# AlenkaF/vaex

Measured on AMD Instinct MI355X. Metric: rows/sec 2D count grid 1e9×f64 + groupby-sum 1e6 keys; HBM GB/s %peak, higher is better.
Workload: dtype f64; 1 GPU; C2 (BASELINE configs[1]): count(binby=[x,y], limits=[[-4,4],[-4,4]], shape=1024) + sum(w), one merged pass; rows_per_gpu=1000000000, parallelism=row-shard x1

## Files before the change

vaex_amd/csrc/engine.hpp:

```cpp
#pragma once
#include <memory>
#include <mutex>
#include <vector>

#include "common.hpp"
#include "hashset.hpp"

struct vh_grid;
struct vh_agg;


namespace vh {

constexpr int MAX_DIM = 16;
constexpr int MAX_FUSED_AGGS = 4;
constexpr uint64_t LDS_FUSED_MAX = 64 * 1024;
constexpr uint64_t LDS_AGG_MAX_BYTES = 96 * 1024;
constexpr int COV_MAX_N = 8;

struct ColumnRef {
    const void *ptr = nullptr;
    uint64_t size = 0;
    int itemsize = 0;
    int loc = VH_LOC_HOST;
// ... 122 lines not shown
    std::vector<int> isz;
    std::vector<uint64_t> off;
    uint64_t chunk = 0, bytes = 0;
    PinnedBuf pinned[2];
    DevBuf dev[2];
    hipEvent_t copied[2] = {nullptr, nullptr}, consumed[2] = {nullptr, nullptr};
    bool pending_copy[2] = {false, false}, pending_use[2] = {false, false};
    std::vector<void *> registered[2];
    ~HostPipe();
    void release_registered(int b);
    void add(const ColumnRef &c);
    void plan(uint64_t chunk_rows);
    void issue(uint64_t ci, uint64_t row0, uint64_t len);
    void wait_copied(int b);
    void mark_consumed(int b);
    int find(const void *ptr) const;
};

struct Workspace {
    DevBuf idx;
    DevBuf cells;
    DevBuf first_part;
    HostPipe pipe;
    ~Workspace();
};

void run_bin(vh_grid *g, vh_agg *const *aggs, int naggs, uint64_t length);
void launch_fused(const BinPlan &plan, FusedAggs &fa, uint64_t n, uint64_t cells, int nd_f64, Workspace &ws);
bool try_tiled(const BinPlan &plan, const FusedAggs &fa, uint64_t n, uint64_t cells, int nd_f64, Workspace &ws);
uint64_t stat_tile_overflow(bool reset);
uint64_t stat_hashagg_overflow(bool reset);
uint64_t stat_set_overflow(bool reset);
uint64_t stat_tile_stream_rounds(bool reset);
bool try_tiled_first(const BinPlan &plan, const AggDev &ad, uint64_t n, uint64_t cells, uint64_t row0, int nd_f64);
uint64_t stat_first_tiled(bool reset);
bool hashagg_bin_set_ordinal(const BinPlan &plan, const FusedAggs &fa, uint64_t n);

}

struct vh_grid {
    std::mutex mu;
    std::vector<vh_binner *> binners;
    std::vector<uint64_t> shapes, strides;
    uint64_t length1d = 1;
    vh::Workspace ws;
};

struct vh_agg {
    vh_grid *grid = nullptr;
    int kind = 0, dtype = VH_F64, flip = 0;
    uint32_t moment = 0;
    int grid_dtype = VH_I64;
    int grid_isz = 8;
    vh::DevBuf g, g2;
    vh::DevBuf s_key, s_row;
    vh::ColumnRef data, data2, mask;
    vh::ColumnRef cols[vh::COV_MAX_N];
    bool has_selection = false;
    bool nu_dirty = false;
    uint64_t L = 0;
    uint64_t nu_n = 0;
    vh::DevBuf nu_cell, nu_val;
};

namespace vh {
void nunique_init(vh_agg *a);
// ... 18 lines not shown
```

vaex_amd/csrc/runtime.hip:

```cpp
#include <map>
#include <mutex>
#include <thread>
#include <cstring>

#include "common.hpp"
#include "engine.hpp"

namespace vh {

static thread_local std::string g_last_error;

void set_error_str(const std::string &s) { g_last_error = s; }
void set_error(const char *fmt, ...) {
    char buf[1024];
    va_list ap;
    va_start(ap, fmt);
    vsnprintf(buf, sizeof(buf), fmt, ap);
    va_end(ap);
    g_last_error = buf;
}

static std::mutex g_mu;
static std::map<int, hipStream_t> g_streams;
static std::map<int, int> g_cus;
// ... 699 lines not shown
    VH_HIP(hipStreamSynchronize(stream()));
    std::lock_guard<std::mutex> lk(g_mu);
    for (auto &kv : g_timing_recs)
        for (auto &p : kv.second.ev) {
            (void)hipEventDestroy(p.first);
            (void)hipEventDestroy(p.second);
        }
    g_timing_recs.clear();
    VH_API_END
}

int vh_timing_read(const char *kernel, uint64_t *launches, double *total_ms) {
    VH_API_BEGIN
    VH_HIP(hipStreamSynchronize(stream()));
    std::lock_guard<std::mutex> lk(g_mu);
    *launches = 0;
    *total_ms = 0;
    auto it = g_timing_recs.find(kernel);
    if (it == g_timing_recs.end()) return VH_OK;
    for (auto &p : it->second.ev) {
        float ms = 0;
        VH_HIP(hipEventElapsedTime(&ms, p.first, p.second));
        *total_ms += ms;
        *launches += 1;
    }
    VH_API_END
}

int vh_stat_read(const char *name, uint64_t *value, int reset) {
    VH_API_BEGIN
    const std::string n = name ? name : "";
    if (n == "tile_overflow_rows") *value = stat_tile_overflow(reset != 0);
    else if (n == "tile_stream_rounds") *value = stat_tile_stream_rounds(reset != 0);
    else if (n == "hashagg_overflow_rows") *value = stat_hashagg_overflow(reset != 0);
    else if (n == "set_overflow_rows") *value = stat_set_overflow(reset != 0);
    else if (n == "first_tiled_chunks") *value = stat_first_tiled(reset != 0);
    else fail(VH_ERR_ARG, "vh_stat_read: unknown statistic '" + n + "'");
    VH_API_END
}

int vh_stream(void **s) {
    VH_API_BEGIN
    *s = (void *)stream();
    VH_API_END
}

static void minmax_result(const DevBuf &keys, double *out_min, double *out_max) {
    thread_local PinnedBuf res_buf;
    res_buf.ensure(16);
    uint64_t *res = res_buf.as<uint64_t>();
    VH_HIP(hipMemcpyAsync(res, keys.ptr, 16, hipMemcpyDeviceToHost, stream()));
    VH_HIP(hipStreamSynchronize(stream()));
    if (res[0] == ~0ULL) {
        *out_min = __builtin_nan("");
        *out_max = __builtin_nan("");
    } else {
        *out_min = f64_from_key(res[0]);
        *out_max = f64_from_key(res[1]);
    }
}

int vh_minmax_sample(const void *data, uint64_t n, int dtype, uint64_t nsample, double *out_min, double *out_max) {
    VH_API_BEGIN
    if (resolve_loc(data, VH_LOC_AUTO) != VH_LOC_DEVICE) throw std::runtime_error("vh_minmax_sample: column not in device memory");
    if (dtype == VH_BOOL) throw std::runtime_error("vh_minmax_sample: bool column");
    const uint64_t ns = std::min(n, nsample);
// ... 67 lines not shown
```

vaex_amd/csrc/tile_plan.hpp:

```cpp
#pragma once
#include <algorithm>
#include <cmath>
#include <vector>

#include "engine.hpp"

namespace vh {

#ifndef VH_TA_THREADS
#define VH_TA_THREADS 512
#endif
#ifndef VH_TA_RPT
#define VH_TA_RPT 8
#endif
#ifndef VH_TB_THREADS
#define VH_TB_THREADS 1024
#endif
#ifndef VH_TILE_LDS_KB
#define VH_TILE_LDS_KB 96
#endif
constexpr int TA_THREADS = VH_TA_THREADS;
constexpr int TA_RPT = VH_TA_RPT;
constexpr int TA_BATCH = TA_THREADS * TA_RPT;
constexpr int TB_THREADS = VH_TB_THREADS;
// ... 42 lines not shown
}

inline bool aligned16(const void *p) { return (reinterpret_cast<uintptr_t>(p) & 15) == 0; }
inline bool aligned8(const void *p) { return (reinterpret_cast<uintptr_t>(p) & 7) == 0; }

struct TileParams {
    uint32_t s_log2, ntiles, flags_mode, nvals;
    uint64_t cells;
    uint32_t W;
    uint32_t pad;
    uint64_t rows_per_wg;
    uint64_t wg_stride;
    const uint32_t *cap;
    const uint64_t *toff;
    uint32_t *fills;
    uint32_t *spill_fill;
    const uint32_t *spill_cap;
    const uint64_t *spill_start;
    uint64_t spill_base;
    void *entries;
    double *values[2];
    int32_t val_slot[MAX_FUSED_AGGS];
    int32_t cnt_slot[MAX_FUSED_AGGS];
    const double *vdata[2];
    uint32_t debug;
    uint32_t vnarrow, vfloat, vsigned;
    uint32_t vpacked;
    int32_t vdt[2];
    void *mmtmp[MAX_FUSED_AGGS];
    uint32_t mgeneric, mmk;
    uint32_t wide, lds_cap;
    uint32_t mm_simple, mm_cnt_nn;
    int32_t mm_off[4];
    uint32_t stream, ncw;
    uint32_t *tab;
    const uint8_t *rowmask;
};

struct TileSwitches {
    bool rowmask = true, f32 = true, narrow = true, stream = true, pack = true;
    uint32_t wide = 7;
    uint64_t wgpad = 0;
    uint32_t debug = 0;
};

struct PassAKernel {
    enum Family { GENERIC, FAST, ORDINAL };
    Family family = GENERIC;
    int nd = 0, nv = 0, sb = 1, ct = VH_F64, vt = VH_F64, dt0 = VH_F64, dt1 = VH_F64;
    bool mk = false, set = false, vn = false;
    const char *scope() const {
        if (family == GENERIC) return "tile_scatter";
        if (family == ORDINAL) return set ? "tile_scatter_set" : "tile_scatter_ord";
        if (ct == VH_I32 || ct == VH_I64) return "tile_scatter_int";
        return ct != vt ? "tile_scatter_mixed" : ct == VH_F32 ? "tile_scatter_f32" : "tile_scatter_f64";
    }
};
const void *pass_a_kernel(const PassAKernel &k);

struct PassBKernel { int nv = 0; bool narrow = false, mm = false, pk = false, mg = false; };
const void *pass_b_kernel(const PassBKernel &k);

struct TilePlan {
    TileParams tp;
    uint32_t lds_off[MAX_FUSED_AGGS];
    uint64_t lds_a, lds_b;
    int sb, vbytes;
    PassAKernel a;
    PassBKernel b;
};

inline bool ord_fast_ok(const BinPlan &plan, const FusedAggs &fa) {
    if (plan.nb != 1) return false;
    const BinnerDev &b = plan.b[0];
    const bool set_ok = b.kind == 2 && (b.dtype == VH_I32 || b.dtype == VH_U32) && !b.set.wide;
    if (!(b.kind == 1 && b.dtype == VH_I32) && !set_ok) return false;
    if (b.flip || b.mask || (reinterpret_cast<uintptr_t>(b.data) & 7)) return false;
    for (int k = 0; k < fa.na; k++) {
        const FusedAgg &a = fa.a[k];
        if (a.mask) return false;
        if (a.kind != VH_AGG_COUNT) {
            if (!a.data) return false;
            const int isz = a.dtype == VH_F64 ? 16 : 2 * dtype_itemsize(a.dtype);
            if (reinterpret_cast<uintptr_t>(a.data) % isz) return false;
        } else if (a.data) {
            bool keyed = false;
            for (int j = 0; j < fa.na; j++)
                if (fa.a[j].kind != VH_AGG_COUNT && fa.a[j].data == a.data) keyed = true;
            if (!keyed) return false;
        }
    }
    return true;
}

// ... 167 lines not shown
    tp.lds_cap = wide ? cap0 + 8 * T : cap0;
    out.lds_a = any_fast ? fast_lds_bytes(nv, T, tp.lds_cap, out.vbytes) : scatter_lds_bytes(nv, T);
    if (out.lds_a > LDS_MAX_BYTES) return false;
    tp.vpacked = (out.vbytes == 4 && nv == 2 && !flags_mode && sw.pack) ? 1u : 0u;

    bool mm = false;
    for (int k = 0; k < fa.na; k++) {
        const FusedAgg &a = fa.a[k];
        mm = mm || is_minmax(a.kind) || a.kind == VH_AGG_SUM_MOMENT;
        if (a.kind == VH_AGG_SUM_MOMENT && a.moment != 2) tp.mgeneric = 1;
        if (is_minmax(a.kind)) tp.mmk |= 1u << k;
    }
    bool simple = mm && !tp.mgeneric && nv == 1 && !vnarrow && !flags_mode;
    int *moff = tp.mm_off;
    moff[0] = moff[1] = moff[2] = moff[3] = -1;
    for (int k = 0; k < fa.na && simple; k++) {
        const FusedAgg &a = fa.a[k];
        const int slot = a.kind == VH_AGG_COUNT ? -1 : tp.val_slot[k];
        int r = -1;
        if (a.kind == VH_AGG_COUNT) {
            r = 0;
            if (tp.cnt_slot[k] == 0) tp.mm_cnt_nn = 1;
            else if (tp.cnt_slot[k] != CNT_ALWAYS) simple = false;
        } else if (a.kind == VH_AGG_SUM && !a.vint && a.dtype == VH_F64 && slot == 0) r = 1;
        else if (a.kind == VH_AGG_MIN && a.dtype == VH_F64 && slot == 0) r = 2;
        else if (a.kind == VH_AGG_MAX && a.dtype == VH_F64 && slot == 0) r = 3;
        else simple = false;
        if (r >= 0) {
            if (moff[r] >= 0) simple = false;
            else moff[r] = (int)out.lds_off[k];
        }
    }
    tp.mm_simple = simple ? 1u : 0u;
    out.b.nv = nv, out.b.pk = nv == 2 && tp.vpacked, out.b.narrow = nv > 0 && (vnarrow || out.b.pk);
    out.b.mm = nv > 0 && mm, out.b.mg = out.b.mm && tp.mgeneric;
    check_pass_a(plan, fa, out);
    return true;
}

struct MetaLayout {
    uint64_t hist;
    uint64_t toff, sstart, scap, sfill, cap;
    uint64_t fills, units, brange;
    uint64_t bytes;
};
struct TileLaunch {
    uint32_t W = 0;
    uint64_t kbat = 0, rows_per_wg = 0, ncw = 0;
    bool stream_layout = false;
    uint64_t stream_stride = 0;
    uint64_t g_min = 1, max_units = 0;
    uint64_t sblocks = 0, bstride = 0;
    MetaLayout meta;
};

inline TileLaunch plan_launch(const TilePlan &pl, uint64_t n, int cus, int blocks_per_cu, const TileSwitches &sw) {
    TileLaunch L;
    const uint32_t T = pl.tp.ntiles;
    const int bpc = std::max(1, std::min(blocks_per_cu, TA_WG_PER_CU));
    const uint32_t W = L.W = std::min<uint32_t>(1024, (uint32_t)cus * bpc);
    const uint64_t nb = (n + TA_BATCH - 1) / TA_BATCH;
    L.kbat = (nb + W - 1) / W;
    L.rows_per_wg = L.kbat * TA_BATCH;
    L.ncw = (L.kbat + pl.sb - 1) / pl.sb;
    L.stream_layout = pl.tp.wide && pl.tp.nvals > 0 && sw.stream && (uint64_t)W * (T + 1) * L.ncw < (1ull << 31);
    L.stream_stride = ((L.rows_per_wg + 7 * L.ncw * T + 8 + 7) & ~uint64_t(7)) + ((sw.wgpad + 7) & ~uint64_t(7));
    const uint64_t wpu = std::max<uint64_t>(1, (uint64_t)TB_THREADS * TB_ROUNDS / std::max<uint64_t>(L.ncw, 1));
    L.g_min = L.stream_layout ? (W + wpu - 1) / wpu : 1;
    L.max_units = (uint64_t)T * L.g_min + 4 * (uint64_t)cus + 16;
    L.sblocks = std::min<uint64_t>(nb, SAMPLE_BLOCKS);
    L.bstride = std::max<uint64_t>(TA_BATCH, n / L.sblocks);
    MetaLayout &m = L.meta;
    uint64_t o = 0;
    auto take = [&](uint64_t bytes) { const uint64_t at = o; o += bytes; return at; };
    m.hist = take(16 * (uint64_t)T);
    m.toff = take(8 * (uint64_t)T);
    m.sstart = take(8 * (uint64_t)T);
    m.scap = take(4 * (uint64_t)T);
    m.sfill = take(4 * (uint64_t)T);
    m.cap = take(4 * (uint64_t)((T + 3) & ~3u));
    m.fills = take(4 * ((uint64_t)T * W + 4 - ((uint64_t)T * W) % 4));
    m.units = take(sizeof(WorkUnit) * L.max_units);
    m.brange = take(8 * (uint64_t)SAMPLE_BLOCKS);
    m.bytes = o;
    return L;
}

inline bool sample_monotone(const uint32_t *brange, uint64_t sblocks) {
    uint64_t up = 0, down = 0;
    for (uint64_t b = 0; b + 1 < sblocks; b++) {
        up += brange[2 * b + 1] > brange[2 * b + 2];
        down += brange[2 * b] < brange[2 * b + 3];
    }
    return sblocks > 8 && std::min(up, down) * 100 <= sblocks;
}

struct TileRegions {
    std::vector<uint32_t> cap, scap;
    std::vector<uint64_t> toff, sstart;
    uint64_t stride = 0, stotal = 0, sampled = 0;
};

inline bool size_regions(const TilePlan &pl, const TileLaunch &L, uint64_t n, const uint64_t *hist, const uint32_t *brange,
                         TileRegions &r) {
    const uint32_t T = pl.tp.ntiles, W = L.W;
    const uint64_t rows_per_wg = L.rows_per_wg, kbat = L.kbat;
    const bool wide = pl.tp.wide != 0, monotone = sample_monotone(brange, L.sblocks);
    uint64_t sampled = 0;
    for (uint32_t t = 0; t < T; t++) sampled += hist[t];
    r.sampled = sampled;
    if (!sampled) return false;
    const uint64_t pad_wg = wide ? 7 * L.ncw : 0;
    r.cap.assign(T, 0), r.scap.assign(T, 0);
    r.toff.assign(T, 0), r.sstart.assign(T, 0);
    uint64_t stride = 0, stotal = 0;
    const double blocks = (double)L.sblocks;
    bool any_clustered = false;
    for (uint32_t t = 0; t < T; t++) {
        const double m = (double)hist[t] / blocks, var_b = std::max(0.0, (double)hist[T + t] / blocks - m * m);
        any_clustered = any_clustered || var_b > 4.0 * m + 1.0;
// ... 78 lines not shown
```

vaex_amd/csrc/tiled.hip:

```cpp
#include <algorithm>
#include <atomic>
#include <cstdio>
#include <cstring>
#include <cmath>
#include <map>
#include <memory>
#include <mutex>
#include <tuple>

#include "binner_dev.hpp"
#include "common.hpp"
#include "engine.hpp"
#include "tile_plan.hpp"

namespace vh {

#ifndef VH_TA_WAVES
#define VH_TA_WAVES 0
#endif
#ifndef VH_TA_NT
#define VH_TA_NT 0
#endif
#ifndef VH_TA_DRAIN
#define VH_TA_DRAIN 1
// ... 1222 lines not shown
    }
}

template <int NV, bool X = false> struct TileRun {
    uint32_t cnt, nn[NV > 0 ? NV : 1];
    double sum[NV > 0 ? NV : 1];
    unsigned long long isum[NV > 0 ? NV : 1];
    double sum2[X && NV > 0 ? NV : 1];
    __device__ void clear() {
        cnt = 0;
#pragma unroll
        for (int s = 0; s < NV; s++) {
            nn[s] = 0;
            sum[s] = 0.0;
            isum[s] = 0;
            if constexpr (X) sum2[s] = 0.0;
        }
    }
    __device__ __attribute__((always_inline)) void add(const TileParams &tp, const double *v) {
        cnt++;
#pragma unroll
        for (int s = 0; s < NV; s++) {
            isum[s] += __builtin_bit_cast(unsigned long long, v[s]);
            if (v[s] == v[s]) {
                nn[s]++;
                sum[s] += v[s];
                if constexpr (X) sum2[s] += v[s] * v[s];
            }

        }
    }
    __device__ __attribute__((always_inline)) void flush(const FusedAggs &fa, const TileParams &tp, unsigned char *lds,
                                                         uint32_t local) const {
#pragma unroll
        for (int k = 0; k < MAX_FUSED_AGGS; k++) {
            if (k >= fa.na) break;
            const int kind = fa.a[k].kind;
            if (kind == VH_AGG_COUNT) {
                const int cs = tp.cnt_slot[k];
                uint32_t c = cs == CNT_ALWAYS || cs == CNT_FLAG ? cnt : 0u;
#pragma unroll
                for (int s = 0; s < NV; s++)
                    if (s == cs) c = nn[s];
                if (c) atomicAdd(reinterpret_cast<uint32_t *>(lds + fa.a[k].lds_off) + local, c);
                continue;
            }
#pragma unroll
            for (int s = 0; s < NV; s++) {
                if (s != tp.val_slot[k]) continue;
                if constexpr (X) {
                    if (kind == VH_AGG_SUM_MOMENT) {
                        if (nn[s]) atomicAdd(reinterpret_cast<double *>(lds + fa.a[k].lds_off) + local, sum2[s]);
                        continue;
                    }
                    if (is_minmax(kind)) continue;
                }
                if (fa.a[k].vint)
                    atomicAdd(reinterpret_cast<unsigned long long *>(lds + fa.a[k].lds_off) + local, isum[s]);
                else if (nn[s])
                    atomicAdd(reinterpret_cast<double *>(lds + fa.a[k].lds_off) + local, sum[s]);
            }
        }
    }
};

constexpr int TB_UNROLL = 8;
// ... 307 lines not shown
#pragma unroll
                                        for (int k = 0; k < MAX_FUSED_AGGS; k++) {
                                            if (!((tp.mmk >> k) & 1u)) continue;
                                            const FusedAgg &a = fa.a[k];
                                            const bool m = a.kind == VH_AGG_MAX;
#pragma unroll
                                            for (int s = 0; s < NV; s++) {
                                                if (s != tp.val_slot[k]) continue;
                                                const uint64_t o = m ? hi[s] : lo[s];
                                                if (o == (m ? 0ull : ~0ull)) continue;
                                                const double r = mm_unokey(a.dtype, o);
                                                if (mm_cell32(a.dtype))
                                                    mm_lds32<false>(reinterpret_cast<uint32_t *>(lds_raw + a.lds_off) + local, a.dtype, m, r);
                                                else
                                                    mm_lds<false>(reinterpret_cast<uint64_t *>(lds_raw + a.lds_off) + local, a.dtype, m, r);
                                            }
                                        }
                                    }
                                }
                            }
                            w0 = (w0 >> 16) | (w1 << 16);
                            w1 = (w1 >> 16) | (w2 << 16);
                            w2 = (w2 >> 16) | (w3 << 16);
                            w3 >>= 16;
#pragma unroll
                            for (int s = 0; s < NV; s++)
#pragma unroll
                                for (int h = 0; h < 7; h++) sv[s][h] = sv[s][h + 1];
                        };
#pragma unroll 1
                        for (uint32_t x = 0; x < rem[j]; x++) entry(x);
                        if (cur != ~0u) run.flush(fa, tp, lds_raw, cur);
                    } else {
                        TileRun<NV, false> run;
                        uint32_t cur = ~0u;
#pragma unroll
                        for (int x = 0; x < 8; x++) {
                            const uint32_t local = (words[x >> 1] >> (16 * (x & 1))) & 0xffffu;
                            if ((uint32_t)x < rem[j] && local != DUMMY_CELL) {
                                if (local != cur) {
                                    if (cur != ~0u) run.flush(fa, tp, lds_raw, cur);
                                    cur = local;
                                    run.clear();
                                }
                                double v[NV > 0 ? NV : 1];
#pragma unroll
                                for (int s = 0; s < NV; s++) v[s] = (x & 1) ? vv[j][s][x >> 1].y : vv[j][s][x >> 1].x;
                                run.add(tp, v);
                            }
                        }
                        if (cur != ~0u) run.flush(fa, tp, lds_raw, cur);
                    }
                }
            } else {
                auto chunk = [&](auto jc) {
                    constexpr int j = decltype(jc)::value;
                    const uint32_t words[4] = {ev[j].x, ev[j].y, ev[j].z, ev[j].w};
#pragma unroll
                    for (int x = 0; x < 8; x++) {
                        if ((uint32_t)x < rem[j]) {
                            double v[NV > 0 ? NV : 1];
#pragma unroll
                            for (int s = 0; s < NV; s++) v[s] = (x & 1) ? vv[j][s][x >> 1].y : vv[j][s][x >> 1].x;
                            const uint32_t local = (words[x >> 1] >> (16 * (x & 1))) & 0xffffu;
                            if (DBG(tp.debug) & 8) asm volatile("" :: "v"(local));
                            else if (local != DUMMY_CELL) reduce_entry<NV, MM>(fa, tp, lds_raw, local, 0xfu, v);
// ... 58 lines not shown
            } else if (is_minmax(fa.a[k].kind)) {
                if constexpr (MM) {
                    const bool mx = fa.a[k].kind == VH_AGG_MAX;
                    const int dt = fa.a[k].dtype;
                    void *tmp = tp.mmtmp[k];
                    if (mm_cell32(dt)) {
                        const uint32_t v = reinterpret_cast<const uint32_t *>(lds_raw + fa.a[k].lds_off)[i];
                        if (v == mm_identity32(dt, mx)) continue;
                        if (!tmp) mm_grid(fa.a[k].grid, c0 + i, dt, mx, mm_cell32_slot(dt, v), false);
                        else if (dt_signed(dt)) mx ? atomicMax(static_cast<int *>(tmp) + c0 + i, (int)v) : atomicMin(static_cast<int *>(tmp) + c0 + i, (int)v);
                        else mx ? atomicMax(static_cast<unsigned *>(tmp) + c0 + i, v) : atomicMin(static_cast<unsigned *>(tmp) + c0 + i, v);
                        continue;
                    }
                    const uint64_t v = reinterpret_cast<const uint64_t *>(lds_raw + fa.a[k].lds_off)[i];
                    if (v == mm_identity(dt, mx)) continue;
                    if (!tmp) mm_grid(fa.a[k].grid, c0 + i, dt, mx, v, true);
                    else if (dt_signed(dt))
                        mx ? atomicMax(static_cast<long long *>(tmp) + c0 + i, (long long)v) : atomicMin(static_cast<long long *>(tmp) + c0 + i, (long long)v);
                    else
                        mx ? atomicMax(static_cast<unsigned long long *>(tmp) + c0 + i, (unsigned long long)v)
                           : atomicMin(static_cast<unsigned long long *>(tmp) + c0 + i, (unsigned long long)v);
                }
            } else if (fa.a[k].vint) {
                const unsigned long long v = reinterpret_cast<const unsigned long long *>(lds_raw + fa.a[k].lds_off)[i];
                if (v) atomicAdd(reinterpret_cast<unsigned long long *>(fa.a[k].grid) + c0 + i, v);
            } else {
                const double v = reinterpret_cast<const double *>(lds_raw + fa.a[k].lds_off)[i];
                if (v != 0.0) atomicAdd(reinterpret_cast<double *>(fa.a[k].grid) + c0 + i, v);
            }
        }
    }
}

#define VH_KP(...) reinterpret_cast<const void *>(__VA_ARGS__)
template <int ND, int NV> static const void *fast_kernel(const PassAKernel &k) {
    constexpr int SBW = fast_sb_nd(NV, ND), SBN = fast_sb_narrow(NV);
#define VH_FAST(CT_, VT_, MK_, SB_, ...) \
    if (k.ct == (CT_) && k.vt == (VT_) && k.mk == (MK_) && k.sb == (SB_)) return VH_KP(k_tile_scatter_f64<ND, NV, SB_, __VA_ARGS__>);
    VH_FAST(VH_F64, VH_F64, true, SBW, double, true)
    VH_FAST(VH_F64, VH_F64, false, 1, double)
    VH_FAST(VH_F64, VH_F64, false, SBW, double)
    VH_FAST(VH_F32, VH_F32, true, SBN, float, true)
    VH_FAST(VH_F32, VH_F32, false, SBN, float)
    if constexpr (NV > 0) {
        VH_FAST(VH_F32, VH_F64, false, SBW, float, false, double)
        VH_FAST(VH_F64, VH_F32, false, SBN, double, false, float)
    }
    if constexpr (ND <= 2) {
        VH_FAST(VH_I32, VH_F64, false, SBW, int32_t, false, double)
        VH_FAST(VH_I64, VH_F64, false, SBW, int64_t, false, double)
        if constexpr (NV > 0) {
            VH_FAST(VH_I32, VH_F32, false, SBN, int32_t, false, float)
            VH_FAST(VH_I64, VH_F32, false, SBN, int64_t, false, float)
        }
    }
#undef VH_FAST
    return nullptr;
}
template <int NV, int SB, bool SET, bool VN> static const void *ord_kernel(const PassAKernel &k) {
    if (k.sb != SB) return nullptr;
#define VH_ORD(a, b, narrow)                                                                   \
    if constexpr ((!SET || (a) == VH_F64 || (a) < 0) && (!VN || narrow)) {                     \
        constexpr int DT1 = (a) < 0 || NV >= 2 ? (b) : VH_F64;                                 \
        if (k.dt0 == (a) && k.dt1 == DT1) return VH_KP(k_tile_scatter_ord<NV, SB, SET, (a), DT1, VN>); \
    }
    VH_ORD_COMBOS(VH_ORD)
// ... 6 lines not shown
            if (k.vn || k.dt0 != VH_F64 || k.dt1 != VH_F64) return nullptr;
            if (k.nv == 0 && k.sb == 1) return VH_KP(k_tile_scatter_ord<0, 1, false, VH_F64, VH_F64, false, true>);
            if (k.nv == 1 && k.sb == fast_sb(1)) return VH_KP(k_tile_scatter_ord<1, fast_sb(1), false, VH_F64, VH_F64, false, true>);
            if (k.nv == 2 && k.sb == fast_sb(2)) return VH_KP(k_tile_scatter_ord<2, fast_sb(2), false, VH_F64, VH_F64, false, true>);
            return nullptr;
        }
        if (k.vn)
            return k.nv == 1 ? ord_kernel<1, fast_sb_narrow(1), false, true>(k) : k.nv == 2 ? ord_kernel<2, fast_sb_narrow(2), false, true>(k) : nullptr;
    }
    if (k.mk || k.vn) return nullptr;
    switch (k.nv) {
    case 0: return ord_kernel<0, 1, SET, false>(k);
    case 1: return k.sb == 1 ? ord_kernel<1, 1, SET, false>(k) : ord_kernel<1, fast_sb(1), SET, false>(k);
    case 2: return k.sb == 1 ? ord_kernel<2, 1, SET, false>(k) : ord_kernel<2, fast_sb(2), SET, false>(k);
    default: return nullptr;
    }
}
template <int NV> static const void *pass_a_kernel_nv(const PassAKernel &k) {
    if (k.family == PassAKernel::FAST)
        return k.nd == 1 ? fast_kernel<1, NV>(k) : k.nd == 2 ? fast_kernel<2, NV>(k) : k.nd == 3 ? fast_kernel<3, NV>(k) : nullptr;
    static const void *const generic[] = {VH_KP(k_tile_scatter<-1, NV>), VH_KP(k_tile_scatter<0, NV>), VH_KP(k_tile_scatter<1, NV>),
                                          VH_KP(k_tile_scatter<2, NV>), VH_KP(k_tile_scatter<3, NV>)};
    return k.sb == 1 && !k.mk && k.nd >= -1 && k.nd <= 3 ? generic[k.nd + 1] : nullptr;
}
const void *pass_a_kernel(const PassAKernel &k) {
    if (k.family == PassAKernel::ORDINAL) return k.set ? ord_kernel_set<true>(k) : ord_kernel_set<false>(k);
    return k.nv == 0 ? pass_a_kernel_nv<0>(k) : k.nv == 1 ? pass_a_kernel_nv<1>(k) : k.nv == 2 ? pass_a_kernel_nv<2>(k) : nullptr;
}
template <int NV, bool NARROW, bool PK> static const void *reduce_kernel(const PassBKernel &k) {
    if (k.mg) return VH_KP(k_tile_reduce<NV, NARROW, true, PK, true>);
    return k.mm ? VH_KP(k_tile_reduce<NV, NARROW, true, PK>) : VH_KP(k_tile_reduce<NV, NARROW, false, PK>);
}
const void *pass_b_kernel(const PassBKernel &k) {
    if (k.nv == 0) return VH_KP(k_tile_reduce<0, false, false>);
    if (k.pk) return reduce_kernel<2, true, true>(k);
    if (k.nv == 1) return k.narrow ? reduce_kernel<1, true, false>(k) : reduce_kernel<1, false, false>(k);
    return k.narrow ? reduce_kernel<2, true, false>(k) : reduce_kernel<2, false, false>(k);
}
static const void *sample_kernel(int nd_f64) {
    static const void *const ks[] = {VH_KP(k_tile_sample<0>), VH_KP(k_tile_sample<1>), VH_KP(k_tile_sample<2>), VH_KP(k_tile_sample<3>)};
    return ks[nd_f64 >= 1 && nd_f64 <= 3 ? nd_f64 : 0];
}
#undef VH_KP

static int blocks_per_cu(const void *kernel, size_t lds) {
    static std::mutex mu;
    static std::map<std::tuple<int, const void *, size_t>, int> cache;
    std::lock_guard<std::mutex> lk(mu);
    const auto key = std::make_tuple(current_device(), kernel, lds);
    auto it = cache.find(key);
    if (it == cache.end()) {
        int v = 0;
        VH_HIP(hipOccupancyMaxActiveBlocksPerMultiprocessor(&v, kernel, TA_THREADS, lds));
        it = cache.emplace(key, v).first;
    }
    return it->second;
}

struct TileScratch {
    std::mutex mu;
    DevBuf entries, values, meta, mmtmp, tab;
};

static TileSwitches read_switches() {
    auto off = [](const char *name) { const char *e = getenv(name); return e && atoi(e) == 0; };
    TileSwitches sw;
    sw.rowmask = !off("VH_TILE_ROWMASK");
    sw.f32 = !off("VH_TILE_F32");
    sw.narrow = !off("VH_TILE_NARROW");
    sw.stream = !off("VH_TILE_STREAM");
    sw.pack = !off("VH_TILE_PACK");
    if (const char *e = getenv("VH_TILE_WIDE")) sw.wide = (uint32_t)atoi(e);
    if (const char *e = getenv("VH_TILE_WGPAD")) sw.wgpad = (uint64_t)strtoull(e, nullptr, 10);
#ifdef VH_ABLATION
    if (const char *e = getenv("VH_TILE_DEBUG")) sw.debug = (uint32_t)atoi(e);
#endif
    return sw;
}
static TileScratch &tile_scratch() {
    static std::mutex g;
    static std::map<int, std::unique_ptr<TileScratch>> m;
    std::lock_guard<std::mutex> lk(g);
    auto &p = m[current_device()];
    if (!p) p = std::make_unique<TileScratch>();
    return *p;
}

static void launch(const void *kernel, unsigned grid, unsigned block, size_t lds, void **args) {
    VH_HIP(hipLaunchKernel(kernel, dim3(grid), dim3(block), args, lds, stream()));
    VH_HIP(hipGetLastError());
}

static std::atomic<uint64_t> g_tile_stream_rounds{0};

static bool try_tiled_core(const BinPlan &plan, const FusedAggs &fa_in, uint64_t n, uint64_t cells, int nd_f64,
                           const uint8_t *rowmask, const TileSwitches &sw) {
    TileScratch &ws = tile_scratch();
    std::lock_guard<std::mutex> ws_lock(ws.mu);
    TilePlan tpl;
    if (!plan_tiles(plan, fa_in, n, cells, nd_f64, rowmask != nullptr, sw, tpl)) return false;
    const void *kernel_a = pass_a_kernel(tpl.a), *kernel_b = pass_b_kernel(tpl.b);
    if (!kernel_a || !kernel_b) fail(VH_ERR_RUNTIME, "tiled binning: the plan names a kernel that is not built");
    const TileLaunch L = plan_launch(tpl, n, cu_count(), blocks_per_cu(kernel_a, tpl.lds_a), sw);
    const uint32_t T = tpl.tp.ntiles, W = L.W;
    const int nv = (int)tpl.tp.nvals;
    hipStream_t st = stream();
    FusedAggs fa = fa_in;
    for (int k = 0; k < fa.na; k++) {
        fa.a[k].lds_off = tpl.lds_off[k];
        if (fa.a[k].kind != VH_AGG_COUNT) tpl.tp.vdata[tpl.tp.val_slot[k]] = fa.a[k].data;
    }
    fa.lds_words = (uint32_t)(tpl.lds_b / 4);
    TileParams &tp = tpl.tp;
    tp.rowmask = rowmask, tp.debug = sw.debug;
    tp.W = W, tp.rows_per_wg = L.rows_per_wg;
    ws.meta.ensure(L.meta.bytes);
    unsigned char *mb = ws.meta.as<unsigned char>();
    auto u32 = [&](uint64_t off) { return reinterpret_cast<uint32_t *>(mb + off); };
    auto u64 = [&](uint64_t off) { return reinterpret_cast<uint64_t *>(mb + off); };
    uint64_t *d_hist = u64(L.meta.hist), *d_hist2 = d_hist + T;
    uint32_t *d_brange = u32(L.meta.brange);
    const WorkUnit *d_units = reinterpret_cast<const WorkUnit *>(mb + L.meta.units);
    tp.cap = u32(L.meta.cap), tp.fills = u32(L.meta.fills), tp.spill_fill = u32(L.meta.sfill), tp.spill_cap = u32(L.meta.scap);
    tp.toff = u64(L.meta.toff), tp.spill_start = u64(L.meta.sstart);

    VH_HIP(hipMemsetAsync(d_hist, 0, 16 * (uint64_t)T, st));
    {
        TimedScope ts("tile_sample");
        BinPlan p = plan;
        uint64_t nn = n, bstride = L.bstride;
        uint32_t s_log2 = tp.s_log2, ntiles = T;
        void *args[] = {&p, &nn, &s_log2, &ntiles, &bstride, &d_hist, &d_hist2, &d_brange};
        launch(sample_kernel(nd_f64), (unsigned)L.sblocks, TA_THREADS, 4 * (size_t)T, args);
    }
    auto setup = [&](uint64_t stride, uint64_t stotal) {
        const uint64_t total = stride * W + stotal + 16;
// ... 44 lines not shown
        uint64_t seen = g_tile_stream_rounds.load(std::memory_order_relaxed);
        while (seen < r && !g_tile_stream_rounds.compare_exchange_weak(seen, r, std::memory_order_relaxed)) {}
    }
    if (!L.stream_layout) setup(reg.stride, reg.stotal);
    char *upl = tstage.as<char>() + dl_bytes;
    auto upload = [&](uint64_t meta_off, const void *src, uint64_t bytes) {
        memcpy(upl, src, bytes);
        VH_HIP(hipMemcpyAsync(mb + meta_off, upl, bytes, hipMemcpyHostToDevice, st));
        upl += (bytes + 15) & ~uint64_t(15);
    };
    upload(L.meta.cap, reg.cap.data(), 4 * (uint64_t)T);
    upload(L.meta.toff, reg.toff.data(), 8 * (uint64_t)T);
    upload(L.meta.sstart, reg.sstart.data(), 8 * (uint64_t)T);
    upload(L.meta.scap, reg.scap.data(), 4 * (uint64_t)T);
    if (!units.empty()) upload(L.meta.units, units.data(), sizeof(WorkUnit) * units.size());
    if (!L.stream_layout) launch_pass_a();
    TimedScope ts("tile_reduce");
    auto mm_size = [&](const FusedAgg &a) { return ((cells * (mm_cell32(a.dtype) ? 4 : 8)) + 255) & ~uint64_t(255); };
    uint64_t mm_bytes = 0;
    for (int k = 0; k < fa.na; k++)
        if (is_minmax(fa.a[k].kind)) mm_bytes += mm_size(fa.a[k]);
    if (tpl.b.mm && mm_bytes <= (1ull << 30)) {
        ws.mmtmp.ensure(mm_bytes + 256);
        uint64_t off = 0;
        for (int k = 0; k < fa.na; k++) {
            if (!is_minmax(fa.a[k].kind)) continue;
            tp.mmtmp[k] = ws.mmtmp.as<char>() + off;
            off += mm_size(fa.a[k]);
            hipLaunchKernelGGL(k_mm_fill, dim3(blocks_for(cells, 256, 8)), dim3(256), 0, st, tp.mmtmp[k], cells,
                               fa.a[k].dtype, (int)(fa.a[k].kind == VH_AGG_MAX));
            VH_HIP(hipGetLastError());
        }
    }
    void *args_b[] = {&fa, &tp, &d_units};
    launch(kernel_b, (unsigned)units.size(), TB_THREADS, tpl.lds_b, args_b);
    for (int k = 0; k < fa.na; k++) {
        if (!tp.mmtmp[k]) continue;
        hipLaunchKernelGGL(k_mm_merge, dim3(blocks_for(cells, 256, 8)), dim3(256), 0, st, fa.a[k].grid, tp.mmtmp[k], cells,
                           fa.a[k].dtype, (int)(fa.a[k].kind == VH_AGG_MAX));
        VH_HIP(hipGetLastError());
    }
    return true;
}

static bool try_tiled_impl(const BinPlan &plan, const FusedAggs &fa_in, uint64_t n, uint64_t cells, int nd_f64) {
    const uint8_t *m = fa_in.na > 0 ? fa_in.a[0].mask : nullptr;
    for (int k = 1; k < fa_in.na && m; k++)
        if (fa_in.a[k].mask != m) m = nullptr;
    for (int d = 0; d < plan.nb && m; d++)
        if (plan.b[d].mask) m = nullptr;
    const TileSwitches sw = read_switches();
    if (m && sw.rowmask) {
        FusedAggs f2 = fa_in;
        for (int k = 0; k < f2.na; k++) f2.a[k].mask = nullptr;
        if (try_tiled_core(plan, f2, n, cells, nd_f64, m, sw)) return true;
    }
    return try_tiled_core(plan, fa_in, n, cells, nd_f64, nullptr, sw);
}

bool try_tiled(const BinPlan &plan, const FusedAggs &fa_in, uint64_t n, uint64_t cells, int nd_f64, Workspace &ws) {
    if (n < (1u << 20) || cells >= (1ull << 40)) return false;
    if ((n & 1) && !fa_in.generic_vals && (nd_f64 > 0 || ord_fast_ok(plan, fa_in))) {
        if (!try_tiled_impl(plan, fa_in, n - 1, cells, nd_f64)) return false;
        BinPlan p1 = plan;
        FusedAggs f1 = fa_in;
        for (int d = 0; d < p1.nb; d++) {
            p1.b[d].data = static_cast<const char *>(p1.b[d].data) + (n - 1) * dtype_itemsize(p1.b[d].dtype);
            if (p1.b[d].mask) p1.b[d].mask += n - 1;
        }
        for (int k = 0; k < f1.na; k++) {
            if (f1.a[k].data) f1.a[k].data += n - 1;
            if (f1.a[k].mask) f1.a[k].mask += n - 1;
        }
        launch_fused(p1, f1, 1, cells, nd_f64, ws);
        return true;
    }
    return try_tiled_impl(plan, fa_in, n, cells, nd_f64);
}

uint64_t stat_tile_overflow(bool reset) {
    unsigned long long v = 0;
    VH_HIP(hipStreamSynchronize(stream()));
    VH_HIP(hipMemcpyFromSymbol(&v, HIP_SYMBOL(d_tile_overflow_rows), sizeof(v)));
    if (reset) {
        const unsigned long long z = 0;
        VH_HIP(hipMemcpyToSymbol(HIP_SYMBOL(d_tile_overflow_rows), &z, sizeof(z)));
    }
    return v;
}

uint64_t stat_tile_stream_rounds(bool reset) {
    return reset ? g_tile_stream_rounds.exchange(0) : g_tile_stream_rounds.load();
}

}
```

Before: 112.4 billion rows/s.

## Add specialized streaming pass-B reduce kernel for count+f64-sum tiled binning

Adds a new tile-reduce kernel, used when the plan is streaming, wide and has one f64 value with only count, non-null count and sum aggregates. Each block does a block-wide prefix scan over segment fills to spread entry chunks evenly across waves. Each wave double-buffers loads of packed 16-bit cell ids and values, and commits run-length-merged counts and sums to LDS with atomics. This is meant to remove the generic per-aggregate flush loop and the load imbalance between segments. It adds more template variants, extra static LDS, and a planner gate, plus debug hooks and a stat counter.

```diff
diff --git a/vaex_amd/csrc/engine.hpp b/vaex_amd/csrc/engine.hpp
--- a/vaex_amd/csrc/engine.hpp
+++ b/vaex_amd/csrc/engine.hpp
@@ -178,6 +178,7 @@
 uint64_t stat_hashagg_overflow(bool reset);
 uint64_t stat_set_overflow(bool reset);
 uint64_t stat_tile_stream_rounds(bool reset);
+uint64_t stat_tile_fast_pass_b(bool reset);
 bool try_tiled_first(const BinPlan &plan, const AggDev &ad, uint64_t n, uint64_t cells, uint64_t row0, int nd_f64);
 uint64_t stat_first_tiled(bool reset);
 bool hashagg_bin_set_ordinal(const BinPlan &plan, const FusedAggs &fa, uint64_t n);
diff --git a/vaex_amd/csrc/runtime.hip b/vaex_amd/csrc/runtime.hip
--- a/vaex_amd/csrc/runtime.hip
+++ b/vaex_amd/csrc/runtime.hip
@@ -755,6 +755,7 @@
     const std::string n = name ? name : "";
     if (n == "tile_overflow_rows") *value = stat_tile_overflow(reset != 0);
     else if (n == "tile_stream_rounds") *value = stat_tile_stream_rounds(reset != 0);
+    else if (n == "tile_fast_pass_b") *value = stat_tile_fast_pass_b(reset != 0);
     else if (n == "hashagg_overflow_rows") *value = stat_hashagg_overflow(reset != 0);
     else if (n == "set_overflow_rows") *value = stat_set_overflow(reset != 0);
     else if (n == "first_tiled_chunks") *value = stat_first_tiled(reset != 0);
diff --git a/vaex_amd/csrc/tile_plan.hpp b/vaex_amd/csrc/tile_plan.hpp
--- a/vaex_amd/csrc/tile_plan.hpp
+++ b/vaex_amd/csrc/tile_plan.hpp
@@ -98,17 +98,21 @@
     uint32_t wide, lds_cap;
     uint32_t mm_simple, mm_cnt_nn;
     int32_t mm_off[4];
+    uint32_t fastb, fb_pad;
+    int32_t fb_off[3], fb_agg[3];
     uint32_t stream, ncw;
     uint32_t *tab;
     const uint8_t *rowmask;
 };
 
 struct TileSwitches {
-    bool rowmask = true, f32 = true, narrow = true, stream = true, pack = true;
+    bool rowmask = true, f32 = true, narrow = true, stream = true, pack = true, fastb = true;
     uint32_t wide = 7;
     uint64_t wgpad = 0;
     uint32_t debug = 0;
 };
+
+TileSwitches read_tile_switches();
 
 struct PassAKernel {
     enum Family { GENERIC, FAST, ORDINAL };
@@ -124,8 +128,9 @@
 };
 const void *pass_a_kernel(const PassAKernel &k);
 
-struct PassBKernel { int nv = 0; bool narrow = false, mm = false, pk = false, mg = false; };
+struct PassBKernel { int nv = 0; bool narrow = false, mm = false, pk = false, mg = false, fast = false, hc = false, hn = false; };
 const void *pass_b_kernel(const PassBKernel &k);
+constexpr size_t FASTB_STATIC_LDS = 2 * TB_SEGS + 4 * (TB_SEGS + 2) + 8 * TB_SEGS + 4 * (TB_THREADS / 64) + 512;
 
 struct TilePlan {
     TileParams tp;
@@ -359,8 +364,23 @@
         }
     }
     tp.mm_simple = simple ? 1u : 0u;
+    bool fb = sw.fastb && sw.stream && tp.wide && !mm && nv == 1 && !vnarrow && !flags_mode &&
+              out.lds_b + FASTB_STATIC_LDS <= LDS_MAX_BYTES;
+    for (int r = 0; r < 3; r++) tp.fb_off[r] = tp.fb_agg[r] = -1;
+    for (int k = 0; k < fa.na && fb; k++) {
+        const FusedAgg &a = fa.a[k];
+        int r = -1;
+        if (a.kind == VH_AGG_COUNT) r = tp.cnt_slot[k] == CNT_ALWAYS ? 0 : tp.cnt_slot[k] == 0 ? 1 : -1;
+        else if (a.kind == VH_AGG_SUM && !a.vint && a.dtype == VH_F64 && tp.val_slot[k] == 0) r = 2;
+        if (r < 0 || tp.fb_off[r] >= 0) fb = false;
+        else tp.fb_off[r] = (int)out.lds_off[k], tp.fb_agg[r] = k;
+    }
+    fb = fb && tp.fb_off[2] >= 0;
+    for (int r = 0; r < 3 && !fb; r++) tp.fb_off[r] = tp.fb_agg[r] = -1;
+    tp.fastb = fb ? 1u : 0u;
     out.b.nv = nv, out.b.pk = nv == 2 && tp.vpacked, out.b.narrow = nv > 0 && (vnarrow || out.b.pk);
     out.b.mm = nv > 0 && mm, out.b.mg = out.b.mm && tp.mgeneric;
+    out.b.fast = fb, out.b.hc = fb && tp.fb_off[0] >= 0, out.b.hn = fb && tp.fb_off[1] >= 0;
     check_pass_a(plan, fa, out);
     return true;
 }
@@ -413,6 +433,12 @@
     return L;
 }
 
+inline PassBKernel pass_b_for(const TilePlan &pl, const TileLaunch &L) {
+    PassBKernel b = pl.b;
+    if (!L.stream_layout) b.fast = b.hc = b.hn = false;
+    return b;
+}
+
 inline bool sample_monotone(const uint32_t *brange, uint64_t sblocks) {
     uint64_t up = 0, down = 0;
     for (uint64_t b = 0; b + 1 < sblocks; b++) {
diff --git a/vaex_amd/csrc/tiled.hip b/vaex_amd/csrc/tiled.hip
--- a/vaex_amd/csrc/tiled.hip
+++ b/vaex_amd/csrc/tiled.hip
@@ -1278,6 +1278,13 @@
     }
     __device__ __attribute__((always_inline)) void flush(const FusedAggs &fa, const TileParams &tp, unsigned char *lds,
                                                          uint32_t local) const {
+        if (DBG(tp.debug) & 8) {
+            uint32_t h = cnt + local;
+#pragma unroll
+            for (int s = 0; s < NV; s++) h += nn[s] + (uint32_t)__double2loint(sum[s]) + (uint32_t)isum[s];
+            if (h == 0x9e3779b9u) atomicAdd(reinterpret_cast<uint32_t *>(lds), h);
+            return;
+        }
 #pragma unroll
         for (int k = 0; k < MAX_FUSED_AGGS; k++) {
             if (k >= fa.na) break;
@@ -1651,6 +1658,17 @@
                         for (uint32_t x = 0; x < rem[j]; x++) entry(x);
                         if (cur != ~0u) run.flush(fa, tp, lds_raw, cur);
                     } else {
+                        if (DBG(tp.debug) & 256) {
+                            uint32_t h = rem[j] + words[0] + words[1] + words[2] + words[3];
+#pragma unroll
+                            for (int s = 0; s < NV; s++)
+#pragma unroll
+                                for (int q = 0; q < 4; q++)
+                                    h += (uint32_t)__double2loint(vv[j][s][q].x) + (uint32_t)__double2hiint(vv[j][s][q].x) +
+                                         (uint32_t)__double2loint(vv[j][s][q].y) + (uint32_t)__double2hiint(vv[j][s][q].y);
+                            if (h == 0x9e3779b9u) atomicAdd(reinterpret_cast<uint32_t *>(lds_raw), h);
+                            continue;
+                        }
                         TileRun<NV, false> run;
                         uint32_t cur = ~0u;
 #pragma unroll
@@ -1775,6 +1793,202 @@
     }
 }
 
+template <bool HC, bool HN>
+__global__ __launch_bounds__(TB_THREADS) void k_tile_reduce_cs(FusedAggs fa, TileParams tp, const WorkUnit *units) {
+    extern __shared__ __align__(16) unsigned char lds_raw[];
+    constexpr uint32_t TBT = TB_THREADS, SEGS = TB_SEGS;
+    constexpr int VU = 2;
+    __shared__ uint64_t s_base[SEGS];
+    __shared__ uint32_t s_pre[SEGS + 2];
+    __shared__ uint16_t s_fill[SEGS];
+    __shared__ uint32_t s_wsum[TBT / 64];
+    static_assert(sizeof(s_base) + sizeof(s_pre) + sizeof(s_fill) + sizeof(s_wsum) + 512 <= FASTB_STATIC_LDS, "the planner's LDS bound");
+    static_assert(TA_BATCH * VH_TA_SB + 8 < 65536, "segment fills are kept in 16 bits");
+    const WorkUnit u = units[blockIdx.x];
+    const uint32_t t = u.tile, T = tp.ntiles, ncw = tp.ncw;
+    const uint32_t nseg = (u.w_end - u.w_begin) * ncw;
+    const uint32_t rounds = (nseg + SEGS - 1) / SEGS;
+    uint32_t pf_f[2] = {0, 0};
+    uint64_t pf_b[2] = {0, 0};
+    auto fetch = [&](uint32_t r) {
+#pragma unroll
+        for (int h = 0; h < 2; h++) {
+            const uint32_t g = r * SEGS + 2 * threadIdx.x + h;
+            pf_f[h] = 0;
+            if (g < nseg) {
+                const uint32_t w = u.w_begin + g / ncw, c = g % ncw;
+                const uint64_t row = ((uint64_t)w * (T + 1) + t) * ncw + c;
+                const uint32_t a = tp.tab[row], e = tp.tab[row + ncw];
+                pf_f[h] = e - a;
+                pf_b[h] = (uint64_t)w * tp.wg_stride + a;
+            }
+        }
+    };
+    auto stream_round = [&]() -> bool {
+        const uint32_t k = 2 * threadIdx.x, lane = threadIdx.x & 63, wave = threadIdx.x >> 6;
+        const uint32_t f0 = pf_f[0], f1 = pf_f[1];
+        const uint32_t ch0 = (f0 + 7) >> 3, ch = ch0 + ((f1 + 7) >> 3);
+        s_fill[k] = (uint16_t)f0;
+        s_fill[k + 1] = (uint16_t)f1;
+        s_base[k] = pf_b[0];
+        s_base[k + 1] = pf_b[1];
+        uint32_t inc = ch;
+#pragma unroll
+        for (int off = 1; off < 64; off <<= 1) {
+            const uint32_t y = __shfl_up(inc, off, 64);
+            if ((int)lane >= off) inc += y;
+        }
+        if (lane == 63) s_wsum[wave] = inc;
+        __syncthreads();
+        uint32_t before = 0, tot = 0;
+#pragma unroll
+        for (uint32_t v = 0; v < TBT / 64; v++) {
+            const uint32_t x = s_wsum[v];
+            before += v < wave ? x : 0u;
+            tot += x;
+        }
+        s_pre[k] = before + inc - ch;
+        s_pre[k + 1] = before + inc - ch + ch0;
+        if (threadIdx.x == 0) s_pre[SEGS] = tot;
+        return (f0 | f1) != 0;
+    };
+    fetch(0);
+    const bool any0 = stream_round();
+    if (!__syncthreads_or(any0 || rounds > 1)) return;
+    {
+        uint4 *lq = reinterpret_cast<uint4 *>(lds_raw);
+        for (uint32_t i = threadIdx.x; i < fa.lds_words / 4; i += TBT) lq[i] = make_uint4(0, 0, 0, 0);
+    }
+    __syncthreads();
+    uint32_t *const cells_c = reinterpret_cast<uint32_t *>(lds_raw + (HC ? tp.fb_off[0] : 0));
+    uint32_t *const cells_n = reinterpret_cast<uint32_t *>(lds_raw + (HN ? tp.fb_off[1] : 0));
+    double *const cells_s = reinterpret_cast<double *>(lds_raw + tp.fb_off[2]);
+    const uint16_t *ent16 = reinterpret_cast<const uint16_t *>(tp.entries);
+    const double *val = tp.values[0];
+    uint32_t sink = 0;
+    auto commit = [&](uint32_t cell, uint32_t rc, uint32_t rn, double rs) __attribute__((always_inline)) {
+        if (DBG(tp.debug) & 8) {
+            sink += cell + rc + rn + (uint32_t)__double2loint(rs);
+            return;
+        }
+        if constexpr (HC) atomicAdd(cells_c + cell, rc);
+        if constexpr (HN) atomicAdd(cells_n + cell, rn);
+        atomicAdd(cells_s + cell, rs);
+    };
+    for (uint32_t r = 0; r < rounds; r++) {
+        if (r > 0) {
+            __syncthreads();
+            stream_round();
+            __syncthreads();
+        }
+        if (r + 1 < rounds) fetch(r + 1);
+        const uint32_t C = s_pre[SEGS];
+        const uint32_t lane = threadIdx.x & 63, nwv = TBT / 64;
+        const uint32_t wave = __builtin_amdgcn_readfirstlane(threadIdx.x >> 6);
+        const uint32_t per_wave = ((C + nwv - 1) / nwv + 63) & ~63u;
+        const uint32_t cb = min(C, wave * per_wave), ce = min(C, cb + per_wave);
+        if (cb >= ce) continue;
+        uint32_t kk = 0;
+        {
+            uint32_t lo = 0, hi = SEGS;
+            while (hi - lo > 1) {
+                const uint32_t mid = (lo + hi) >> 1;
+                if (s_pre[mid] <= cb) lo = mid;
+                else hi = mid;
+            }
+            kk = lo;
+        }
+        uint32_t p0 = s_pre[kk], p1 = s_pre[kk + 1];
+        auto load = [&](uint32_t c0, uint4 (&ev)[VU], double2 (&vv)[VU][4], uint32_t (&rem)[VU]) __attribute__((always_inline)) {
+#pragma unroll
+            for (int j = 0; j < VU; j++) {
+                const uint32_t c = c0 + j * 64 + lane;
+                const uint32_t cc = c < ce ? c : ce - 1;
+                while (p1 <= cc) {
+                    kk++;
+                    p0 = p1;
+                    p1 = s_pre[kk + 1];
+                }
+                const uint32_t q = (cc - p0) * 8;
+                const uint64_t e = s_base[kk] + q;
+                rem[j] = c < ce ? min(8u, (uint32_t)s_fill[kk] - q) : 0u;
+                ev[j] = *reinterpret_cast<const uint4 *>(ent16 + e);
+#pragma unroll
+                for (int h = 0; h < 4; h++) vv[j][h] = *reinterpret_cast<const double2 *>(val + e + 2 * h);
+            }
+        };
+        auto apply = [&](const uint4 (&ev)[VU], const double2 (&vv)[VU][4], const uint32_t (&rem)[VU]) __attribute__((always_inline)) {
+#pragma unroll
+            for (int j = 0; j < VU; j++) {
+                const uint32_t words[4] = {ev[j].x, ev[j].y, ev[j].z, ev[j].w};
+                const double vx[8] = {vv[j][0].x, vv[j][0].y, vv[j][1].x, vv[j][1].y, vv[j][2].x, vv[j][2].y, vv[j][3].x, vv[j][3].y};
+                if (DBG(tp.debug) & 256) {
+#pragma unroll
+                    for (int x = 0; x < 8; x++) sink += (words[x >> 1] ^ (uint32_t)__double2loint(vx[x])) + (uint32_t)__double2hiint(vx[x]);
+                    sink += rem[j];
+                    continue;
+                }
+                uint32_t cur = ~0u, rc = 0, rn = 0;
+                double rs = 0.0;
+#pragma unroll
+                for (int x = 0; x < 8; x++) {
+                    const uint32_t local = (words[x >> 1] >> (16 * (x & 1))) & 0xffffu;
+                    if ((uint32_t)x >= rem[j] || local == DUMMY_CELL) continue;
+                    if (local != cur) {
+                        if (cur != ~0u) commit(cur, rc, rn, rs);
+                        cur = local;
+                        rc = rn = 0;
+                        rs = 0.0;
+                    }
+                    const double v = vx[x];
+                    const bool ok = v == v;
+                    rc++;
+                    rn += ok ? 1u : 0u;
+                    rs += ok ? v : 0.0;
+                }
+                if (cur != ~0u) commit(cur, rc, rn, rs);
+            }
+        };
+        constexpr uint32_t STEP = 64 * VU;
+        uint4 ev_a[VU], ev_b[VU];
+        double2 vv_a[VU][4], vv_b[VU][4];
+        uint32_t rem_a[VU], rem_b[VU];
+        load(cb, ev_a, vv_a, rem_a);
+        for (uint32_t c0 = cb;; c0 += 2 * STEP) {
+            const bool more_b = c0 + STEP < ce;
+            if (more_b) load(c0 + STEP, ev_b, vv_b, rem_b);
+            apply(ev_a, vv_a, rem_a);
+            if (!more_b) break;
+            const bool more_a = c0 + 2 * STEP < ce;
+            if (more_a) load(c0 + 2 * STEP, ev_a, vv_a, rem_a);
+            apply(ev_b, vv_b, rem_b);
+            if (!more_a) break;
+        }
+    }
+    __syncthreads();
+    if (DBG(tp.debug) & (8 | 256)) {
+        if (sink == 0x9e3779b9u) cells_c[0] = sink;
+    }
+    if (DBG(tp.debug) & 16) return;
+    const uint64_t c0 = (uint64_t)t << tp.s_log2;
+    const uint32_t ncell = (uint32_t)min((uint64_t)1 << tp.s_log2, tp.cells - c0);
+    if constexpr (HC) {
+        unsigned long long *grid = reinterpret_cast<unsigned long long *>(fa.a[tp.fb_agg[0]].grid) + c0;
+        for (uint32_t i = threadIdx.x; i < ncell; i += TBT)
+            if (const uint32_t v = cells_c[i]) atomicAdd(grid + i, (unsigned long long)v);
+    }
+    if constexpr (HN) {
+        unsigned long long *grid = reinterpret_cast<unsigned long long *>(fa.a[tp.fb_agg[1]].grid) + c0;
+        for (uint32_t i = threadIdx.x; i < ncell; i += TBT)
+            if (const uint32_t v = cells_n[i]) atomicAdd(grid + i, (unsigned long long)v);
+    }
+    double *grid = reinterpret_cast<double *>(fa.a[tp.fb_agg[2]].grid) + c0;
+    for (uint32_t i = threadIdx.x; i < ncell; i += TBT) {
+        const double v = cells_s[i];
+        if (v != 0.0) atomicAdd(grid + i, v);
+    }
+}
+
 #define VH_KP(...) reinterpret_cast<const void *>(__VA_ARGS__)
 template <int ND, int NV> static const void *fast_kernel(const PassAKernel &k) {
     constexpr int SBW = fast_sb_nd(NV, ND), SBN = fast_sb_narrow(NV);
@@ -1847,6 +2061,11 @@
     return k.mm ? VH_KP(k_tile_reduce<NV, NARROW, true, PK>) : VH_KP(k_tile_reduce<NV, NARROW, false, PK>);
 }
 const void *pass_b_kernel(const PassBKernel &k) {
+    if (k.fast) {
+        if (k.nv != 1 || k.narrow || k.mm || k.pk) return nullptr;
+        return k.hc ? (k.hn ? VH_KP(k_tile_reduce_cs<true, true>) : VH_KP(k_tile_reduce_cs<true, false>))
+                    : (k.hn ? VH_KP(k_tile_reduce_cs<false, true>) : VH_KP(k_tile_reduce_cs<false, false>));
+    }
     if (k.nv == 0) return VH_KP(k_tile_reduce<0, false, false>);
     if (k.pk) return reduce_kernel<2, true, true>(k);
     if (k.nv == 1) return k.narrow ? reduce_kernel<1, true, false>(k) : reduce_kernel<1, false, false>(k);
@@ -1885,6 +2104,7 @@
     sw.narrow = !off("VH_TILE_NARROW");
     sw.stream = !off("VH_TILE_STREAM");
     sw.pack = !off("VH_TILE_PACK");
+    sw.fastb = !off("VH_TILE_FASTB");
     if (const char *e = getenv("VH_TILE_WIDE")) sw.wide = (uint32_t)atoi(e);
     if (const char *e = getenv("VH_TILE_WGPAD")) sw.wgpad = (uint64_t)strtoull(e, nullptr, 10);
 #ifdef VH_ABLATION
@@ -1892,6 +2112,7 @@
 #endif
     return sw;
 }
+TileSwitches read_tile_switches() { return read_switches(); }
 static TileScratch &tile_scratch() {
     static std::mutex g;
     static std::map<int, std::unique_ptr<TileScratch>> m;
@@ -1907,6 +2128,7 @@
 }
 
 static std::atomic<uint64_t> g_tile_stream_rounds{0};
+static std::atomic<uint64_t> g_tile_fast_pass_b{0};
 
 static bool try_tiled_core(const BinPlan &plan, const FusedAggs &fa_in, uint64_t n, uint64_t cells, int nd_f64,
                            const uint8_t *rowmask, const TileSwitches &sw) {
@@ -1914,9 +2136,11 @@
     std::lock_guard<std::mutex> ws_lock(ws.mu);
     TilePlan tpl;
     if (!plan_tiles(plan, fa_in, n, cells, nd_f64, rowmask != nullptr, sw, tpl)) return false;
-    const void *kernel_a = pass_a_kernel(tpl.a), *kernel_b = pass_b_kernel(tpl.b);
-    if (!kernel_a || !kernel_b) fail(VH_ERR_RUNTIME, "tiled binning: the plan names a kernel that is not built");
+    const void *kernel_a = pass_a_kernel(tpl.a);
+    if (!kernel_a) fail(VH_ERR_RUNTIME, "tiled binning: the plan names a kernel that is not built");
     const TileLaunch L = plan_launch(tpl, n, cu_count(), blocks_per_cu(kernel_a, tpl.lds_a), sw);
+    const void *kernel_b = pass_b_kernel(pass_b_for(tpl, L));
+    if (!kernel_b) fail(VH_ERR_RUNTIME, "tiled binning: the plan names a kernel that is not built");
     const uint32_t T = tpl.tp.ntiles, W = L.W;
     const int nv = (int)tpl.tp.nvals;
     hipStream_t st = stream();
@@ -2027,6 +2251,7 @@
             VH_HIP(hipGetLastError());
         }
     }
+    if (pass_b_for(tpl, L).fast) g_tile_fast_pass_b.fetch_add(1, std::memory_order_relaxed);
     void *args_b[] = {&fa, &tp, &d_units};
     launch(kernel_b, (unsigned)units.size(), TB_THREADS, tpl.lds_b, args_b);
     for (int k = 0; k < fa.na; k++) {
@@ -2084,6 +2309,10 @@
     return v;
 }
 
+uint64_t stat_tile_fast_pass_b(bool reset) {
+    return reset ? g_tile_fast_pass_b.exchange(0) : g_tile_fast_pass_b.load();
+}
+
 uint64_t stat_tile_stream_rounds(bool reset) {
     return reset ? g_tile_stream_rounds.exchange(0) : g_tile_stream_rounds.load();
 }
```

Measured after the change: 113.2 billion rows/s (median of 6 runs). About the same (+0.7%).
